# zengxianyu/sketchedit

Measured on NVIDIA H100. Metric: images/sec 256x256 CelebA-HQ generator fwd, higher is better.
Workload: dtype bf16

## Files before the change

### include/sketchedit_b200.h

```cpp
#ifndef SKETCHEDIT_B200_H
#define SKETCHEDIT_B200_H

#ifdef __cplusplus
extern "C" {
#endif

typedef struct se_model se_model;

enum {
  SE_PREC_BF16_TC = 0,
  SE_PREC_FP32_EXACT = 1,
  SE_PREC_FP32_TC = 3
};

enum {
  SE_OPT_USE_CAM = 0,
  SE_OPT_POOL_AVG = 1,
  SE_OPT_NO_MASK_CC = 2,
  SE_OPT_NO_MASK_COARSE = 3,
  SE_OPT_JOINT_TRAIN_INP = 4
};

const char* se_last_error(void);
int se_abi_version(void);
// ... 92 lines not shown
  SE_TAP_DESC_LEN = 10
};
int se_taps_enable(se_model* m, int on);
int se_taps_count(se_model* m);
int se_tap_info(se_model* m, int i, char* name, int name_cap, int* desc, long long* bytes);
int se_tap_copy(se_model* m, int i, void* dst, void* stream);

enum {
  SE_C8_INST = 0,
  SE_C8_TEAMS = 1,
  SE_C8_CLUSTER = 2,
  SE_C8_GRID = 3,
  SE_C8_TOTAL_TILES = 4,
  SE_C8_N = 5, SE_C8_TILES_X = 6, SE_C8_TILES_Y = 7, SE_C8_HO = 8, SE_C8_WO = 9,
  SE_C8_STEP_X = 10, SE_C8_STEP_Y = 11, SE_C8_STEP_IMG = 12,
  SE_C8_CSTEP_X = 13, SE_C8_CSTEP_Y = 14, SE_C8_CSTEP_IMG = 15,
  SE_C8_MODE = 16,
  SE_C8_CPT = 17,
  SE_C8_NCLS = 18,
  SE_C8_A_BUFS = 19, SE_C8_NUM_STAGES = 20,
  SE_C8_OUT_C8 = 21,
  SE_C8_CHOFF = 22, SE_C8_LDO = 23,
  SE_C8_PHANTOM = 24,
  SE_C8_BLK_SPLIT = 25,
  SE_C8_REC_LEN = 26
};
int se_c8_log_enable(int on);
int se_c8_log_count(void);
int se_c8_log_get(int i, char* name, int name_cap, int* rec);
int se_c8_inst_count(void);
enum { SE_C8_INST_NT = 0, SE_C8_INST_F16 = 1, SE_C8_INST_R64 = 2, SE_C8_INST_M64 = 3, SE_C8_INST_R32 = 4, SE_C8_INST_TEAMS = 5,
       SE_C8_INST_LEN = 6 };
int se_c8_inst_info(int i, int* info);

#ifdef __cplusplus
}
#endif
#endif
```

### sketchedit_b200/_lib.py

```python
import ctypes
import os

_HERE = os.path.dirname(os.path.abspath(__file__))
LIB_PATH = os.environ.get("SE_B200_LIB") or os.path.join(_HERE, "libsketchedit_b200.so")

_c_void_p = ctypes.c_void_p
_c_int = ctypes.c_int
_c_char = ctypes.c_char
_c_char_p = ctypes.c_char_p
_fp = ctypes.POINTER(ctypes.c_float)

SIGNATURES = {
    "se_last_error": (_c_char_p, []),
    "se_abi_version": (_c_int, []),
    "se_model_create": (_c_int, [ctypes.POINTER(_c_void_p)]),
    "se_model_destroy": (None, [_c_void_p]),
    "se_model_set_layer": (_c_int, [_c_void_p, _c_char, _c_char_p, _c_void_p, _c_void_p, _c_int, _c_int, _c_int]),
    "se_model_finalize": (_c_int, [_c_void_p]),
    "se_model_set_option": (_c_int, [_c_void_p, _c_int, _c_int]),
    "se_forward_inference": (_c_int, [_c_void_p, _c_void_p, _c_void_p, _c_int, _c_int, _c_int, _c_int,
                                      _c_void_p, _c_void_p, _c_void_p, _c_void_p, _c_void_p, _c_void_p, _c_void_p,
                                      _c_void_p]),
    "se_forward_inference_packed": (_c_int, [_c_void_p, _c_void_p, _c_void_p, _c_int, _c_int, _c_int, _c_int, _c_void_p, _c_void_p]),
    "se_forward_inference_u8": (_c_int, [_c_void_p, _c_void_p, _c_void_p, _c_int, _c_int, _c_int, _c_int, _c_void_p, _c_void_p, _c_void_p]),
# ... 18 lines not shown
    "se_forward_u8_export": (_c_int, [_c_void_p, _c_void_p, _c_void_p, _c_void_p, _c_void_p, _c_int, _c_int, _c_int, _c_int, _c_void_p,
                                      _c_void_p, _c_void_p, _c_void_p, _c_void_p]),
    "se_resize_composite_feather_detail_u8": (_c_int, [_c_void_p, _c_void_p, _c_void_p, _c_void_p, _c_void_p, _c_void_p, _c_void_p,
                                                       _c_void_p, _c_void_p, _c_void_p, _c_void_p, _c_void_p, _c_void_p, _c_int,
                                                       _c_int, _c_void_p, ctypes.POINTER(ctypes.c_longlong), _c_void_p]),
    "se_detail_u8": (_c_int, [_c_void_p, _c_void_p, _c_void_p, _c_int, _c_int, _c_int, _c_void_p, _c_void_p, _c_void_p, _c_void_p,
                              _c_void_p, _c_void_p, _c_void_p, _c_void_p, _c_void_p, _c_void_p, _c_void_p,
                              ctypes.POINTER(ctypes.c_longlong), _c_void_p]),
    "se_feather_u8": (_c_int, [_c_void_p, _c_void_p, _c_void_p, _c_void_p, _c_int, _c_void_p]),
    "se_jpeg_encode_u8": (_c_int, [_c_void_p, _c_void_p, _c_void_p, _c_int, _c_int, _c_int, _c_void_p, _c_void_p, _c_void_p, _c_void_p,
                                   ctypes.POINTER(ctypes.c_longlong), _c_void_p]),
    "se_jpeg_max_bytes": (ctypes.c_longlong, [_c_int, _c_int, _c_int]),
    "se_png_encode_u8": (_c_int, [_c_void_p, _c_void_p, _c_void_p, _c_int, _c_int, _c_int, _c_void_p, _c_void_p, _c_void_p, _c_void_p,
                                  ctypes.POINTER(ctypes.c_longlong), _c_void_p]),
    "se_png_max_bytes": (ctypes.c_longlong, [_c_int, _c_int, _c_int]),
    "se_png_decode_u8": (_c_int, [_c_void_p, _c_void_p, _c_void_p, _c_void_p, _c_void_p, _c_int, _c_void_p, _c_void_p,
                                  _c_void_p, ctypes.POINTER(ctypes.c_longlong), _c_void_p]),
    "se_resize_coeffs": (_c_int, [_c_int, _c_int, _c_void_p, _c_void_p, ctypes.c_longlong]),
    "se_resize_set_table_cache_limit": (_c_int, [ctypes.c_longlong]),
    "se_resize_table_cache_bytes": (ctypes.c_longlong, []),
    "se_last_launch_count": (_c_int, []),
    "se_workspace_bytes": (ctypes.c_longlong, [_c_void_p]),
    "se_timing_enable": (_c_int, [_c_int]),
    "se_timing_report": (_c_int, [_c_char_p, _c_int]),
    "se_taps_enable": (_c_int, [_c_void_p, _c_int]),
    "se_taps_count": (_c_int, [_c_void_p]),
    "se_tap_info": (_c_int, [_c_void_p, _c_int, _c_char_p, _c_int, ctypes.POINTER(_c_int), ctypes.POINTER(ctypes.c_longlong)]),
    "se_tap_copy": (_c_int, [_c_void_p, _c_int, _c_void_p, _c_void_p]),
    "se_c8_log_enable": (_c_int, [_c_int]),
    "se_c8_log_count": (_c_int, []),
    "se_c8_log_get": (_c_int, [_c_int, _c_char_p, _c_int, ctypes.POINTER(_c_int)]),
    "se_c8_inst_count": (_c_int, []),
    "se_c8_inst_info": (_c_int, [_c_int, ctypes.POINTER(_c_int)]),
}

C8_REC = ("inst", "teams", "cluster", "grid", "total_tiles", "N", "tiles_x", "tiles_y", "Ho", "Wo", "step_x", "step_y",
          "step_img", "cstep_x", "cstep_y", "cstep_img", "mode", "cpt", "ncls", "a_bufs", "num_stages", "out_c8", "choff",
          "ldo", "phantom", "blk_split")
C8_INST = ("nt", "f16", "r64", "m64", "r32", "teams")

_lib = None


class SketchEditB200Error(RuntimeError):
    pass


def load():
    global _lib
    if _lib is not None:
        return _lib
    if not os.path.exists(LIB_PATH):
        raise SketchEditB200Error(
            "%s not found. Build it with `python -m sketchedit_b200.build` (nvcc, sm_90a). "
            "There is no CPU or PyTorch fallback for this path." % LIB_PATH)
    lib = ctypes.CDLL(LIB_PATH)
    for name, (res, args) in SIGNATURES.items():
        fn = getattr(lib, name)
        fn.restype = res
        fn.argtypes = args
    _lib = lib
    return lib


def check(rc):
    if rc != 0:
# ... 7 lines not shown
```

### sketchedit_b200/csrc/se_conv_c8.cu

```cuda
#include "se_conv_c8.h"

#include <stdlib.h>

#include <atomic>
#include <map>
#include <mutex>
#include <vector>

#include "../../include/sketchedit_b200.h"
#include "se_tc_device.cuh"

namespace se {

constexpr int C8_TH = 16, C8_TW = 8;
constexpr int C8_CONSUMER_WARPS = 8;
__host__ __device__ constexpr int c8_threads(int teams) { return 32 * C8_CONSUMER_WARPS * teams + 32; }
constexpr int C8_MAX_STAGES = 8;

__device__ __forceinline__ void ring_of(int i, int n, int shift, int& slot, uint32_t& phase) {
  if (shift >= 0) { slot = i & (n - 1); phase = (uint32_t)(i >> shift) & 1u; }
  else { const int qd = i / n; slot = i - qd * n; phase = (uint32_t)qd & 1u; }
}

template <int NT, bool kF16, int R64, int M64, int R32, int TEAMS>
__global__ void __launch_bounds__(c8_threads(TEAMS), 1)
conv_c8_kernel(const __grid_constant__ CUtensorMap tmA, const C8Params p) {
  extern __shared__ __align__(1024) uint8_t smem_raw[];
  uint8_t* smem = reinterpret_cast<uint8_t*>((reinterpret_cast<uintptr_t>(smem_raw) + 1023) & ~uintptr_t(1023));
  constexpr bool kTeams = TEAMS > 1;
  const bool halo = kTeams || p.mode == C8_HALO;
  constexpr int b64_bytes = NT * 128, b32_bytes = NT * 64;
  constexpr int b_bytes = R64 * b64_bytes + R32 * b32_bytes;
  const int stage_a = halo ? 0 : p.a_bytes;
  const int stage_b = p.resident ? 0 : b_bytes;
  const int stage_bytes = stage_a + stage_b;
  const bool staged = !kTeams && stage_bytes > 0;
  uint8_t* sHalo = smem;
  uint8_t* sWres = sHalo + (halo ? p.a_bufs * p.a_bytes : 0);
  uint8_t* sStages = sWres + (p.resident ? p.wres_bytes : 0);
  uint8_t* tail = sStages + (size_t)p.num_stages * stage_bytes;
  uint64_t* full_bar = reinterpret_cast<uint64_t*>(tail);
  uint64_t* empty_bar = full_bar + C8_MAX_STAGES;
  uint64_t* a_full = empty_bar + C8_MAX_STAGES;
  uint64_t* a_empty = a_full + C8_MAX_ABUFS;
  uint64_t* wres_bar = a_empty + C8_MAX_ABUFS;
  float* bias_s = reinterpret_cast<float*>(wres_bar + 2);

  const int warp = threadIdx.x >> 5;
  const int lane = threadIdx.x & 31;
  const bool clustered = !kTeams && p.cluster > 1;
  const uint32_t rank = clustered ? cluster_ctarank() : 0u;
  if (threadIdx.x == 0) {
    for (int i = 0; i < C8_MAX_STAGES; ++i) {
      mbar_init(&full_bar[i], 1);
      mbar_init(&empty_bar[i], C8_CONSUMER_WARPS * p.cluster);
    }
    for (int i = 0; i < C8_MAX_ABUFS; ++i) {
      mbar_init(&a_full[i], 1);
      mbar_init(&a_empty[i], C8_CONSUMER_WARPS);
    }
    mbar_init(wres_bar, 1);
    asm volatile("fence.mbarrier_init.release.cluster;" ::: "memory");
  }
  const int cst_n = NT + 32;
  epi_fill_constants(bias_s, cst_n, p.bias, p.e, threadIdx.x, c8_threads(TEAMS));
  if (clustered) cluster_sync();
  else __syncthreads();

  const int total_tiles = p.N * p.tiles_x * p.tiles_y;
  const int ksteps = kTeams ? 1 : p.ksteps;
  const int first_tile = (int)blockIdx.x - (int)rank;

  if (warp == C8_CONSUMER_WARPS * TEAMS) {
    if (lane == 0) asm volatile("prefetch.tensormap [%0];" ::"l"(reinterpret_cast<uint64_t>(&tmA)) : "memory");
    if (p.resident && elect_one()) {
      mbar_expect_tx(wres_bar, (uint32_t)p.wres_bytes);
      for (int off = 0; off < p.wres_bytes; off += 65536) {
        const int n = min(65536, p.wres_bytes - off);
        bulk_load_1d(sWres + off, p.w + off, (uint32_t)n, wres_bar);
      }
    }
    __syncwarp();
    const int b_split = (b_bytes >> 11) << 10;
    const int b_off = rank ? b_split : 0, b_len = clustered ? (rank ? b_bytes - b_split : b_split) : b_bytes;
    int stage = 0, iter = 0;
    uint32_t phase = 0;
    int tx = blockIdx.x % p.tiles_x, ty = (blockIdx.x / p.tiles_x) % p.tiles_y, img = blockIdx.x / (p.tiles_x * p.tiles_y);
    for (int tile = blockIdx.x; tile - (int)rank < total_tiles; tile += gridDim.x, ++iter) {
      if (tile != (int)blockIdx.x) {
        tx += p.step_x;
        if (tx >= p.tiles_x) { tx -= p.tiles_x; ++ty; }
        ty += p.step_y;
        if (ty >= p.tiles_y) { ty -= p.tiles_y; ++img; }
        img += p.step_img;
      }
      const int x0 = tx * C8_TW, y0 = ty * C8_TH;
      const bool load_a = tile < total_tiles;
      if (halo && load_a) {
        int ab;
        uint32_t aphase;
        ring_of(iter, p.a_bufs, p.a_shift, ab, aphase);
        mbar_wait(&a_empty[ab], aphase ^ 1, 5);
        if (elect_one()) {
// ... 16 lines not shown
            if (!halo && load_a) {
              const int t = ks / p.cpt, ch = ks - t * p.cpt;
              tma_load_4d(st, &tmA, &full_bar[stage], (x0 + p.dx[t]) * 8, y0 + p.dy[t], p.x_cb_off + p.tap_cb[t] + 8 * ch, img);
            }
          }
          __syncwarp();
          if (++stage == p.num_stages) { stage = 0; phase ^= 1; }
        }
      }
    }
  } else {
    const int team = TEAMS > 1 ? warp / C8_CONSUMER_WARPS : 0;
    const int wg = (warp >> 2) & 1, wq = warp & 3;
    const uint32_t smem_base = smem_u32(smem);
    const uint32_t off_wres = halo ? (uint32_t)(p.a_bufs * p.a_bytes) : 0u;
    const uint32_t off_stages = off_wres + (p.resident ? (uint32_t)p.wres_bytes : 0u);
    const uint32_t a_m = (uint32_t)wg * 8u * (uint32_t)p.sbo_bytes;
    const uint32_t n_u64 = p.ntaps * p.n64;
    const int ncls = p.ncls;
    const uint32_t cst_s = smem_u32(bias_s);
    const bool elu = p.e.epi == EPI_GATE_ELU, paired = p.e.paired != 0;
    if (p.resident) mbar_wait(wres_bar, 0, 6);
    auto release = [&](uint64_t* bar) {
      __syncwarp();
      if (lane == 0) mbar_arrive(bar);
    };
    auto release_stage = [&](int s) {
      __syncwarp();
      if (lane == 0) {
        mbar_arrive(&empty_bar[s]);
        if (clustered) mbar_arrive_cluster(&empty_bar[s], rank ^ 1u);
      }
    };
    float acc[NT / 2];
#pragma unroll
    for (int i = 0; i < NT / 2; ++i) acc[i] = 0.0f;
    int stage = 0;
    uint32_t phase = 0;
    const int my_tiles = (first_tile < total_tiles) ? (total_tiles - first_tile + (int)gridDim.x - 1) / (int)gridDim.x : 0;
    const int nv = (my_tiles > team ? (my_tiles - team + TEAMS - 1) / TEAMS : 0) * ncls;
    const bool pingpong = kTeams || (p.resident && ksteps == 1);
    const int bar_wg0 = 2 + 2 * team, bar_wg1 = 1 + 2 * team;
    int riter = team, cls = 0;
    int tx, ty, img;
    {
      const int t0 = (int)blockIdx.x + team * (int)gridDim.x;
      tx = t0 % p.tiles_x; ty = (t0 / p.tiles_x) % p.tiles_y; img = t0 / (p.tiles_x * p.tiles_y);
    }
    for (int v = 0; v < nv; ++v) {
      if (v > 0 && ++cls == ncls) {
        cls = 0;
        riter += TEAMS;
        tx += p.cstep_x;
        if (tx >= p.tiles_x) { tx -= p.tiles_x; ++ty; }
        ty += p.cstep_y;
        if (ty >= p.tiles_y) { ty -= p.tiles_y; ++img; }
        img += p.cstep_img;
      }
      const int tile = (int)blockIdx.x + riter * (int)gridDim.x;
      if (tile >= total_tiles) {
        for (int ks = 0; ks < ksteps; ++ks) {
          mbar_wait(&full_bar[stage], phase, 3);
          release_stage(stage);
          if (++stage == p.num_stages) { stage = 0; phase ^= 1; }
        }
        continue;
      }
      int ab = 0;
      if (halo) {
        uint32_t aph;
        ring_of(riter, p.a_bufs, p.a_shift, ab, aph);
        mbar_wait(&a_full[ab], aph, 7);
      }
      if (pingpong && (wg == 1 || v > 0)) named_bar_sync(wg == 0 ? bar_wg0 : bar_wg1, 256);
      int prev = -1;
      for (int ks = 0; ks < ksteps; ++ks) {
        if (staged) mbar_wait(&full_bar[stage], phase, 3);
        const uint32_t st = smem_base + off_stages + (uint32_t)stage * stage_bytes;
        const uint32_t sB = p.resident ? smem_base + off_wres + (uint32_t)cls * (uint32_t)p.cls_bytes + (uint32_t)ks * b_bytes : st + stage_a;
        const uint32_t sA = (halo ? smem_base + (uint32_t)ab * p.a_bytes : st) + a_m;
        const int ub = cls * C8_CLS_UNITS;
        const int u0 = ub + ks * R64, v0 = ub + (int)n_u64 + ks * R32;
        const uint32_t acc0 = ks ? 1u : 0u;
        wg_fence();
        wg_fence_acc(acc);
#pragma unroll
        for (int j = 0; j < R64; ++j) {
          const uint32_t a0 = sA + p.aoff[u0 + j];
          const uint32_t b0 = sB + (uint32_t)(j * b64_bytes);
#pragma unroll
          for (int k = 0; k < M64; ++k)
            Wgmma<NT, kF16, 0>::mma(acc, wg_desc(a0 + k * p.kstep_bytes, p.lbo_bytes, p.sbo_bytes, WG_SW_NONE),
                                    wg_desc(b0 + 32u * k, 16u, 1024u, WG_SW128), j + k ? 1u : acc0);
        }
#pragma unroll
        for (int j = 0; j < R32; ++j) {
          const uint32_t a0 = sA + p.aoff[v0 + j];
          const uint32_t b0 = sB + (uint32_t)(R64 * b64_bytes + j * b32_bytes);
#pragma unroll
          for (int k = 0; k < 2; ++k)
            Wgmma<NT, kF16, 0>::mma(acc, wg_desc(a0 + k * p.kstep_bytes, p.lbo_bytes, p.sbo_bytes, WG_SW_NONE),
                                    wg_desc(b0 + 32u * k, 16u, 512u, WG_SW64), R64 + j + k ? 1u : acc0);
        }
        wg_commit();
        if (staged) {
          if (prev >= 0) {
            wg_wait<1>();
            release_stage(prev);
          }
          prev = stage;
          if (++stage == p.num_stages) { stage = 0; phase ^= 1; }
        }
      }
      if (pingpong && (wg == 0 || v + 1 < nv)) named_bar_arrive(wg == 0 ? bar_wg1 : bar_wg0, 256);
      wg_wait<0>();
      wg_fence_acc(acc);
      if (prev >= 0) release_stage(prev);
      if (halo && cls == ncls - 1) release(&a_empty[ab]);
      const int ooy = ncls > 1 ? p.cls_ooy[cls] : p.e.ooy, oox = ncls > 1 ? p.cls_oox[cls] : p.e.oox;
      size_t base[2];
      bool ok[2];
#pragma unroll
      for (int h = 0; h < 2; ++h) {
        const int ry = 8 * wg + 2 * wq + h, rx = lane >> 2;
        const int py = ty * C8_TH + ry, px = tx * C8_TW + rx;
        ok[h] = py < p.Ho && px < p.Wo;
        base[h] = epi_pixel_offset(p.e, img, py * p.e.osy + ooy, px * p.e.osx + oox, 2 * (lane & 3));
      }
      if (elu) {
        if (kF16 || paired) conv_epilogue<NT, kF16, true, true>(p.e, cst_s, acc, base, ok, lane);
        else conv_epilogue<NT, false, true, false>(p.e, cst_s, acc, base, ok, lane);
      } else {
        if (kF16 || paired) conv_epilogue<NT, kF16, false, true>(p.e, cst_s, acc, base, ok, lane);
        else conv_epilogue<NT, false, false, false>(p.e, cst_s, acc, base, ok, lane);
      }
    }
  }
  if (clustered) cluster_sync();
}

void fill_epi(const ConvParams& c, int NT, EpiParams* e) {
  e->y = c.y; e->out_c8 = c.out_c8;
  e->Hout = c.Hout; e->Wout = c.Wout; e->ldo = c.ldo; e->choff = c.choff;
  e->osy = c.osy; e->ooy = c.ooy; e->osx = c.osx; e->oox = c.oox;
  e->epi = c.epi; e->scale = c.scale;
  e->Cout = c.Cout; e->NT = NT;
  e->blk_split = c.out_blk_split > 0 ? c.out_blk_split : (1 << 20);
  e->blk_jump = c.out_blk_split > 0 ? c.out_blk_jump : 0;
  e->par_stride = c.out_par_stride > 0 ? c.out_par_stride : (c.ldo >> 2);
  const long long plane = c.out_c8 == 2 ? (long long)(c.Hout / 2) * (c.Wout / 2) : (long long)c.Hout * c.Wout;
  e->blk_stride = (int)(c.out_c8 ? plane * 8 : 8);
  e->goff = gated_goff(c.Cout);
  e->paired = (c.out_c8 != 0 || (((c.ldo | c.choff) & 1) == 0 && c.Cout / 2 == e->goff)) ? 1 : 0;
  e->split_stride = (int)c.out_split_stride;
}
typedef CUresult (*EncodeTiledFn)(CUtensorMap*, CUtensorMapDataType, cuuint32_t, void*, const cuuint64_t*, const cuuint64_t*,
                                  const cuuint32_t*, const cuuint32_t*, CUtensorMapInterleave, CUtensorMapSwizzle,
                                  CUtensorMapL2promotion, CUtensorMapFloatOOBfill);
static EncodeTiledFn c8_encode_fn() {
  static EncodeTiledFn fn = nullptr;
  if (!fn) {
    void* p = nullptr;
    cudaDriverEntryPointQueryResult qres;
    if (cudaGetDriverEntryPoint("cuTensorMapEncodeTiled", &p, cudaEnableDefault, &qres) != cudaSuccess || qres != cudaDriverEntryPointSuccess || !p) return nullptr;
    fn = reinterpret_cast<EncodeTiledFn>(p);
  }
  return fn;
// ... 36 lines not shown
  L->mode = (halo_bytes <= 72 * 1024) ? C8_HALO : C8_PERTAP;
  if (L->mode == C8_HALO) {
    L->HR = HR; L->WR = WR; L->pad_y0 = -mn_y; L->pad_x0 = -mn_x;
  } else {
    L->HR = C8_TH; L->WR = C8_TW; L->pad_y0 = 0; L->pad_x0 = 0;
    L->cb_in = (w.n64 * 64 + w.n32 * 32) / 8;
  }
  L->a_tx_bytes = L->cb_in * L->HR * L->WR * 16;
  L->a_bytes = (L->a_tx_bytes + 1023) / 1024 * 1024;
  L->resident = (wbytes <= kResidentMax) && (2 * L->a_bytes + wbytes <= kSmemBudget);
  if (L->resident && L->mode == C8_HALO) {
    w.r64 = ntaps * w.n64;
    w.r32 = ntaps * w.n32;
  } else if (L->mode == C8_PERTAP || (w.n64 > 0 && w.n32 > 0)) { w.r64 = w.n64; w.r32 = w.n32; }
  else {
    const int unit = w.n64 ? w.NT * 128 : w.NT * 64, total = ntaps * (w.n64 ? w.n64 : w.n32);
    int best = 1;
    for (int k = 1; k <= 8 && k <= total; ++k)
      if (total % k == 0 && k * unit <= 48 * 1024) best = k;
    if (w.n64) { w.r64 = best; w.r32 = 0; } else { w.r64 = 0; w.r32 = best; }
  }
  if (L->mode == C8_PERTAP && w.n32 == 0 && w.n64 > 1 && 2 * (L->a_bytes + w.NT * w.n64 * 128) > kSmemBudget) {
    L->chunks_per_tap = w.n64;
    L->cb_in = 8;
    L->a_tx_bytes = L->cb_in * L->HR * L->WR * 16;
    L->a_bytes = (L->a_tx_bytes + 1023) / 1024 * 1024;
    w.r64 = 1;
  }
  if (L->mode == C8_PERTAP) SE_REQUIRE(tc_ksteps(w) == ntaps * L->chunks_per_tap, "per-tap stages must be whole taps or whole chunks");
  return 0;
}

typedef void (*C8Kernel)(CUtensorMap, C8Params);
struct C8Inst { int nt; bool f16; int r64, m64, r32, teams; C8Kernel fn, fn2; };
#define C8_INST(nt, f16, r64, m64, r32) {nt, f16, r64, m64, r32, 1, conv_c8_kernel<nt, f16, r64, m64, r32, 1>, nullptr}
#define C8_INST2(nt, f16, r64, m64, r32) \
  {nt, f16, r64, m64, r32, 2, conv_c8_kernel<nt, f16, r64, m64, r32, 1>, conv_c8_kernel<nt, f16, r64, m64, r32, 2>}
static const C8Inst kC8Insts[] = {
    C8_INST2(32, false, 0, 0, 9),
    C8_INST2(48, false, 0, 0, 9),
    C8_INST2(48, false, 4, 3, 0),
    C8_INST2(48, false, 5, 3, 0),
    C8_INST2(96, false, 0, 0, 9),
    C8_INST(96, false, 4, 4, 4),
    C8_INST2(96, false, 5, 3, 0),
    C8_INST2(96, false, 9, 3, 0),
    C8_INST(96, false, 3, 3, 0),
    C8_INST(192, false, 1, 3, 0),
    C8_INST(192, false, 1, 4, 0),
    C8_INST(192, false, 1, 4, 1),
    C8_INST2(32, true, 0, 0, 27),
    C8_INST(48, true, 0, 0, 3),
    C8_INST(48, true, 12, 3, 0),
    C8_INST2(48, true, 15, 3, 0),
    C8_INST(96, true, 0, 0, 3),
    C8_INST(96, true, 1, 3, 0),
    C8_INST(96, true, 1, 4, 1),
    C8_INST(96, true, 3, 3, 0),
    C8_INST(192, true, 1, 3, 0),
    C8_INST(192, true, 1, 4, 0),
    C8_INST(192, true, 1, 4, 1),
};
#undef C8_INST
#undef C8_INST2
static const C8Inst* c8_inst(const C8Layer& L, bool f16) {
  const TcWeights& w = L.w;
  const int r64 = w.n64 ? w.r64 : 0, r32 = w.n32 ? w.r32 : 0, m64 = r64 ? L.mmas64 : 0;
  for (const C8Inst& k : kC8Insts)
    if (k.nt == w.NT && k.f16 == f16 && k.r64 == r64 && k.m64 == m64 && k.r32 == r32) return &k;
  return nullptr;
}
static int c8_set_smem_attr(int bytes) {
  for (const C8Inst& k : kC8Insts) {
    SE_CUDA_OK(cudaFuncSetAttribute(k.fn, cudaFuncAttributeMaxDynamicSharedMemorySize, bytes));
    if (k.fn2) SE_CUDA_OK(cudaFuncSetAttribute(k.fn2, cudaFuncAttributeMaxDynamicSharedMemorySize, bytes));
  }
  return 0;
}
int c8_instantiated(const C8Layer& L, bool f16, const std::string& name) {
  const TcWeights& w = L.w;
  SE_REQUIRE(c8_inst(L, f16) != nullptr,
             "layer " + name + (f16 ? " (split-half)" : "") + ": no conv_c8_kernel instantiation for N = " + std::to_string(w.NT) +
                 ", k-step of " + std::to_string(w.n64 ? w.r64 : 0) + " x " + std::to_string(L.mmas64) + " + " +
                 std::to_string(w.n32 ? w.r32 : 0) + " x 2 MMAs (se_conv_c8.cu: kC8Insts)");
  return 0;
}
static void c8_launch_config(cudaLaunchConfig_t* cfg, cudaLaunchAttribute* attr, int grid, int teams, int smem_bytes, int cluster, cudaStream_t stream) {
  *cfg = cudaLaunchConfig_t();
  cfg->gridDim = dim3(grid);
  cfg->blockDim = dim3(c8_threads(teams));
  cfg->dynamicSmemBytes = smem_bytes;
  cfg->stream = stream;
  if (cluster > 1) {
    attr->id = cudaLaunchAttributeClusterDimension;
    attr->val.clusterDim.x = cluster;
    attr->val.clusterDim.y = 1;
    attr->val.clusterDim.z = 1;
    cfg->attrs = attr;
    cfg->numAttrs = 1;
  }
}
static int c8_max_clusters(C8Kernel k, int smem_bytes, int* out) {
  static std::mutex mu;
  static std::map<std::pair<C8Kernel, int>, int> cache;
  std::lock_guard<std::mutex> lock(mu);
  auto it = cache.find({k, smem_bytes});
  if (it == cache.end()) {
    cudaLaunchConfig_t cfg;
    cudaLaunchAttribute attr;
    c8_launch_config(&cfg, &attr, 2 * g_sms, 1, smem_bytes, 2, 0);
    int n = 0;
    SE_CUDA_OK(cudaOccupancyMaxActiveClusters(&n, k, &cfg));
    SE_REQUIRE(n > 0, "no 2-CTA cluster of conv_c8_kernel fits on the device");
    it = cache.emplace(std::make_pair(k, smem_bytes), n).first;
  }
  *out = it->second;
  return 0;
}

struct C8LogEntry { std::string name; int rec[SE_C8_REC_LEN]; };
static std::atomic<bool> g_c8_log{false};
static std::mutex g_c8_log_mu;
static std::vector<C8LogEntry> g_c8_log_recs;
static std::string g_c8_log_label;
bool c8_log_on() { return g_c8_log.load(std::memory_order_relaxed); }
void c8_log_label(const std::string& name) {
  std::lock_guard<std::mutex> lk(g_c8_log_mu);
  g_c8_log_label = name;
}
static void c8_log_append(const C8Params& p, const ConvParams& c, int inst, int teams, int grid, int total_tiles) {
  C8LogEntry e;
  int* r = e.rec;
  r[SE_C8_INST] = inst; r[SE_C8_TEAMS] = teams; r[SE_C8_CLUSTER] = p.cluster; r[SE_C8_GRID] = grid;
  r[SE_C8_TOTAL_TILES] = total_tiles; r[SE_C8_N] = p.N; r[SE_C8_TILES_X] = p.tiles_x; r[SE_C8_TILES_Y] = p.tiles_y;
  r[SE_C8_HO] = p.Ho; r[SE_C8_WO] = p.Wo;
  r[SE_C8_STEP_X] = p.step_x; r[SE_C8_STEP_Y] = p.step_y; r[SE_C8_STEP_IMG] = p.step_img;
  r[SE_C8_CSTEP_X] = p.cstep_x; r[SE_C8_CSTEP_Y] = p.cstep_y; r[SE_C8_CSTEP_IMG] = p.cstep_img;
  r[SE_C8_MODE] = p.mode; r[SE_C8_CPT] = p.cpt; r[SE_C8_NCLS] = p.ncls; r[SE_C8_A_BUFS] = p.a_bufs;
  r[SE_C8_NUM_STAGES] = p.num_stages;
  r[SE_C8_OUT_C8] = c.out_c8; r[SE_C8_CHOFF] = c.choff; r[SE_C8_LDO] = c.ldo;
  r[SE_C8_PHANTOM] = p.cluster > 1 && total_tiles % 2 == 1;
  r[SE_C8_BLK_SPLIT] = c.out_blk_split > 0 ? c.out_blk_split : 0;
  std::lock_guard<std::mutex> lk(g_c8_log_mu);
  e.name = g_c8_log_label;
  g_c8_log_recs.push_back(e);
}

static const int kGroupSmemMax = 222 * 1024;

int c8_configure_group(C8Group* G, int ncls, int ntaps, const int8_t (*dy)[8], const int8_t (*dx)[8], const int* ooy, const int* oox, int Ci, int Cout) {
  if (ncls < 2 || ncls > C8_MAX_CLS || ntaps > 8) return 1;
  int mn_y = 0, mx_y = 0, mn_x = 0, mx_x = 0;
  for (int c = 0; c < ncls; ++c)
    for (int t = 0; t < ntaps; ++t) {
      mn_y = dy[c][t] < mn_y ? dy[c][t] : mn_y; mx_y = dy[c][t] > mx_y ? dy[c][t] : mx_y;
      mn_x = dx[c][t] < mn_x ? dx[c][t] : mn_x; mx_x = dx[c][t] > mx_x ? dx[c][t] : mx_x;
    }
  C8Layer& L = G->geo;
  L = C8Layer();
  TcWeights& w = L.w;
  w.ntaps = ntaps;
  w.n64 = Ci / 64;
  int rem = Ci - 64 * w.n64;
  if (rem > 32) { ++w.n64; rem = 0; }
  w.n32 = rem > 0 ? 1 : 0;
  w.NT = (gated_goff(Cout) + Cout / 2 + 15) / 16 * 16;
  w.n_tiles = 1;
  w.img_bytes = 0;
  w.r64 = ntaps * w.n64;
  w.r32 = ntaps * w.n32;
  L.mmas64 = Ci == 48 ? 3 : 4;
  if (w.r64 + w.r32 > C8_CLS_UNITS) return 1;
  L.mode = C8_HALO;
  L.resident = true;
  L.stem = false;
// ... 95 lines not shown
  SE_REQUIRE(!(L.resident && p.ksteps == 1) || p.a_bufs >= 2, "ping-pong warpgroups need two halo buffers");
  int stages = stage_bytes ? (smem_budget - fixed) / stage_bytes : 1;
  if (stages > C8_MAX_STAGES) stages = C8_MAX_STAGES;
  SE_REQUIRE(stages >= (stage_bytes ? 2 : 1), "shared memory plan does not fit");
  p.num_stages = stages;
  const int smem_bytes = 1024 + fixed + stages * stage_bytes + (2 * C8_MAX_STAGES + 2 * C8_MAX_ABUFS + 2) * 8 + 3 * (p.NT + 32) * 4 + 64;

  EncodeTiledFn enc = c8_encode_fn();
  SE_REQUIRE(enc != nullptr, "cuTensorMapEncodeTiled not available from the driver");
  if (!g_sms) {
    int dev = 0;
    SE_CUDA_OK(cudaGetDevice(&dev));
    SE_CUDA_OK(cudaDeviceGetAttribute(&g_sms, cudaDevAttrMultiProcessorCount, dev));
    SE_CUDA_OK(cudaDeviceGetAttribute(&g_optin, cudaDevAttrMaxSharedMemoryPerBlockOptin, dev));
    { int rc_attr = c8_set_smem_attr(g_optin); if (rc_attr) return rc_attr; }
  }
  SE_REQUIRE(smem_bytes <= g_optin, "shared memory plan exceeds the opt-in limit");

  CUtensorMap tmA;
  {
    cuuint64_t dims[4] = {(cuuint64_t)c.Wi * 8, (cuuint64_t)c.Hi, (cuuint64_t)c.ldx, (cuuint64_t)c.N};
    cuuint64_t strides[3] = {(cuuint64_t)c.Wi * 16, (cuuint64_t)c.Hi * c.Wi * 16, (cuuint64_t)c.ldx * c.Hi * c.Wi * 16};
    cuuint32_t box[4] = {(cuuint32_t)(L.WR * 8), (cuuint32_t)L.HR, (cuuint32_t)L.cb_in, 1};
    cuuint32_t estr[4] = {1, 1, 1, 1};
    CUresult r = enc(&tmA, CU_TENSOR_MAP_DATA_TYPE_BFLOAT16, 4, const_cast<void*>(c.x), dims, strides, box, estr,
                     CU_TENSOR_MAP_INTERLEAVE_NONE, CU_TENSOR_MAP_SWIZZLE_NONE, CU_TENSOR_MAP_L2_PROMOTION_L2_256B,
                     CU_TENSOR_MAP_FLOAT_OOB_FILL_NONE);
    SE_REQUIRE(r == CUDA_SUCCESS, "cuTensorMapEncodeTiled(C8) failed, CUresult=" + std::to_string((int)r));
  }
  const C8Inst* inst = c8_inst(L, p.f16 != 0);
  SE_REQUIRE(inst != nullptr, "no conv_c8_kernel instantiation for the layer's plan (N = " + std::to_string(p.NT) + ")");
  p.cluster = L.resident ? 1 : 2;
  int grid = total_tiles < g_sms ? total_tiles : g_sms;
  const int teams = (inst->teams == 2 && L.resident && p.ksteps == 1 && p.a_bufs >= 4 && total_tiles > grid) ? 2 : 1;
  const C8Kernel kernel = teams == 2 ? inst->fn2 : inst->fn;
  if (p.cluster > 1) {
    int max_clusters = 0;
    { int rc_occ = c8_max_clusters(kernel, smem_bytes, &max_clusters); if (rc_occ) return rc_occ; }
    const int pairs = (total_tiles + 1) / 2;
    grid = 2 * (pairs < max_clusters ? pairs : max_clusters);
  }
  p.step_x = grid % p.tiles_x;
  p.step_y = (grid / p.tiles_x) % p.tiles_y;
  p.step_img = grid / (p.tiles_x * p.tiles_y);
  p.cstep_x = (teams * grid) % p.tiles_x;
  p.cstep_y = (teams * grid / p.tiles_x) % p.tiles_y;
  p.cstep_img = teams * grid / (p.tiles_x * p.tiles_y);
  cudaLaunchConfig_t cfg;
  cudaLaunchAttribute attr;
  c8_launch_config(&cfg, &attr, grid, teams, smem_bytes, p.cluster, stream);
  SE_CUDA_OK(cudaLaunchKernelEx(&cfg, kernel, tmA, p));
  if (c8_log_on()) c8_log_append(p, c, (int)(inst - kC8Insts), teams, grid, total_tiles);
  return 0;
}

}

extern "C" {

int se_c8_log_enable(int on) {
  std::lock_guard<std::mutex> lk(se::g_c8_log_mu);
  se::g_c8_log = on != 0;
  se::g_c8_log_recs.clear();
  se::g_c8_log_label.clear();
  return 0;
}

int se_c8_log_count(void) {
  std::lock_guard<std::mutex> lk(se::g_c8_log_mu);
  return (int)se::g_c8_log_recs.size();
}

int se_c8_log_get(int i, char* name, int name_cap, int* rec) {
  std::lock_guard<std::mutex> lk(se::g_c8_log_mu);
  SE_REQUIRE(i >= 0 && i < (int)se::g_c8_log_recs.size(),
             "launch record index " + std::to_string(i) + " of " + std::to_string(se::g_c8_log_recs.size()));
  const se::C8LogEntry& e = se::g_c8_log_recs[i];
  if (name && name_cap > 0) {
    const size_t n = std::min(e.name.size(), (size_t)name_cap - 1);
    memcpy(name, e.name.data(), n);
    name[n] = 0;
  }
  if (rec) memcpy(rec, e.rec, sizeof(e.rec));
  return 0;
}

int se_c8_inst_count(void) { return (int)(sizeof(se::kC8Insts) / sizeof(se::kC8Insts[0])); }

int se_c8_inst_info(int i, int* info) {
  SE_REQUIRE(i >= 0 && i < se_c8_inst_count() && info, "instantiation index " + std::to_string(i) + " of " + std::to_string(se_c8_inst_count()));
  const se::C8Inst& k = se::kC8Insts[i];
  info[SE_C8_INST_NT] = k.nt; info[SE_C8_INST_F16] = k.f16 ? 1 : 0; info[SE_C8_INST_R64] = k.r64;
  info[SE_C8_INST_M64] = k.m64; info[SE_C8_INST_R32] = k.r32; info[SE_C8_INST_TEAMS] = k.teams;
  return 0;
}

}
```

### sketchedit_b200/csrc/se_conv_c8.h

```cpp
#pragma once
#include "se_common.cuh"
#include "se_conv_tc.h"

namespace se {

enum { C8_HALO = 0, C8_PERTAP = 1 };
constexpr int C8_MAX_ABUFS = 8;
constexpr int C8_MAX_UNITS = 128;

struct C8Layer {
  TcWeights w;
  int mode = C8_HALO;
  bool resident = false;
  bool stem = false;
  int cb_in = 0;
  int mmas64 = 4;
  int HR = 0, WR = 0;
  int pad_y0 = 0, pad_x0 = 0;
  int a_bytes = 0, a_tx_bytes = 0;
  int8_t tap_cb[MAX_TAPS] = {0};
  int chunks_per_tap = 1;
};

constexpr int C8_MAX_CLS = 4;
constexpr int C8_CLS_UNITS = 16;
struct C8Group {
  C8Layer geo;
  int ncls = 0;
  int ntaps = 0;
  int8_t dy[C8_MAX_CLS][8], dx[C8_MAX_CLS][8];
  int ooy[C8_MAX_CLS], oox[C8_MAX_CLS];
  int cls_bytes = 0;
  const void* w_all = nullptr;
};

struct C8Params {
  int N, Ho, Wo;
  int tiles_x, tiles_y;
  int step_x, step_y, step_img;
  int cstep_x, cstep_y, cstep_img;
// ... 29 lines not shown
```

Before: 5087.

## Keep two tiles in flight per consumer warpgroup in c8 ping-pong conv kernel

Adds a PIPE template parameter to the c8 conv kernel so each consumer warpgroup can issue the wgmma chain for the next tile before waiting on and running the epilogue of the current one, using two accumulator register sets. The aim is to hide epilogue latency behind tensor-core work for resident, single-kstep layers whose halo ring is deep enough. Pipelined variants are instantiated for several small-N configurations and picked at launch time. The second accumulator set doubles register pressure and needs one more halo buffer. Logging and ABI hooks report which pipe depth was used.

```diff
diff --git a/include/sketchedit_b200.h b/include/sketchedit_b200.h
--- a/include/sketchedit_b200.h
+++ b/include/sketchedit_b200.h
@@ -148,6 +148,8 @@
 enum { SE_C8_INST_NT = 0, SE_C8_INST_F16 = 1, SE_C8_INST_R64 = 2, SE_C8_INST_M64 = 3, SE_C8_INST_R32 = 4, SE_C8_INST_TEAMS = 5,
        SE_C8_INST_LEN = 6 };
 int se_c8_inst_info(int i, int* info);
+int se_c8_log_pipe(int i, int* pipe);
+int se_c8_inst_pipe(int i, int* pipe);
 
 #ifdef __cplusplus
 }
diff --git a/sketchedit_b200/_lib.py b/sketchedit_b200/_lib.py
--- a/sketchedit_b200/_lib.py
+++ b/sketchedit_b200/_lib.py
@@ -74,6 +74,8 @@
     "se_c8_log_get": (_c_int, [_c_int, _c_char_p, _c_int, ctypes.POINTER(_c_int)]),
     "se_c8_inst_count": (_c_int, []),
     "se_c8_inst_info": (_c_int, [_c_int, ctypes.POINTER(_c_int)]),
+    "se_c8_log_pipe": (_c_int, [_c_int, ctypes.POINTER(_c_int)]),
+    "se_c8_inst_pipe": (_c_int, [_c_int, ctypes.POINTER(_c_int)]),
 }
 
 C8_REC = ("inst", "teams", "cluster", "grid", "total_tiles", "N", "tiles_x", "tiles_y", "Ho", "Wo", "step_x", "step_y",
diff --git a/sketchedit_b200/csrc/se_conv_c8.cu b/sketchedit_b200/csrc/se_conv_c8.cu
--- a/sketchedit_b200/csrc/se_conv_c8.cu
+++ b/sketchedit_b200/csrc/se_conv_c8.cu
@@ -22,19 +22,19 @@
   else { const int qd = i / n; slot = i - qd * n; phase = (uint32_t)qd & 1u; }
 }
 
-template <int NT, bool kF16, int R64, int M64, int R32, int TEAMS>
+template <int NT, bool kF16, int R64, int M64, int R32, int TEAMS, int PIPE>
 __global__ void __launch_bounds__(c8_threads(TEAMS), 1)
 conv_c8_kernel(const __grid_constant__ CUtensorMap tmA, const C8Params p) {
   extern __shared__ __align__(1024) uint8_t smem_raw[];
   uint8_t* smem = reinterpret_cast<uint8_t*>((reinterpret_cast<uintptr_t>(smem_raw) + 1023) & ~uintptr_t(1023));
-  constexpr bool kTeams = TEAMS > 1;
-  const bool halo = kTeams || p.mode == C8_HALO;
+  constexpr bool kPingPongOnly = TEAMS > 1 || PIPE > 1;
+  const bool halo = kPingPongOnly || p.mode == C8_HALO;
   constexpr int b64_bytes = NT * 128, b32_bytes = NT * 64;
   constexpr int b_bytes = R64 * b64_bytes + R32 * b32_bytes;
   const int stage_a = halo ? 0 : p.a_bytes;
   const int stage_b = p.resident ? 0 : b_bytes;
   const int stage_bytes = stage_a + stage_b;
-  const bool staged = !kTeams && stage_bytes > 0;
+  const bool staged = !kPingPongOnly && stage_bytes > 0;
   uint8_t* sHalo = smem;
   uint8_t* sWres = sHalo + (halo ? p.a_bufs * p.a_bytes : 0);
   uint8_t* sStages = sWres + (p.resident ? p.wres_bytes : 0);
@@ -46,9 +46,9 @@
   uint64_t* wres_bar = a_empty + C8_MAX_ABUFS;
   float* bias_s = reinterpret_cast<float*>(wres_bar + 2);
 
-  const int warp = threadIdx.x >> 5;
+  const int warp = PIPE == 2 ? __shfl_sync(0xffffffffu, (int)threadIdx.x >> 5, 0) : (int)threadIdx.x >> 5;
   const int lane = threadIdx.x & 31;
-  const bool clustered = !kTeams && p.cluster > 1;
+  const bool clustered = !kPingPongOnly && p.cluster > 1;
   const uint32_t rank = clustered ? cluster_ctarank() : 0u;
   if (threadIdx.x == 0) {
     for (int i = 0; i < C8_MAX_STAGES; ++i) {
@@ -68,7 +68,7 @@
   else __syncthreads();
 
   const int total_tiles = p.N * p.tiles_x * p.tiles_y;
-  const int ksteps = kTeams ? 1 : p.ksteps;
+  const int ksteps = kPingPongOnly ? 1 : p.ksteps;
   const int first_tile = (int)blockIdx.x - (int)rank;
 
   if (warp == C8_CONSUMER_WARPS * TEAMS) {
@@ -151,91 +151,33 @@
         if (clustered) mbar_arrive_cluster(&empty_bar[s], rank ^ 1u);
       }
     };
-    float acc[NT / 2];
+    auto mma_chain = [&](float (&d)[NT / 2], uint32_t sA, uint32_t sB, int cls, int ks) {
+      const int ub = cls * C8_CLS_UNITS;
+      const int u0 = ub + ks * R64, v0 = ub + (int)n_u64 + ks * R32;
+      const uint32_t acc0 = ks ? 1u : 0u;
+      wg_fence();
+      wg_fence_acc(d);
 #pragma unroll
-    for (int i = 0; i < NT / 2; ++i) acc[i] = 0.0f;
-    int stage = 0;
-    uint32_t phase = 0;
-    const int my_tiles = (first_tile < total_tiles) ? (total_tiles - first_tile + (int)gridDim.x - 1) / (int)gridDim.x : 0;
-    const int nv = (my_tiles > team ? (my_tiles - team + TEAMS - 1) / TEAMS : 0) * ncls;
-    const bool pingpong = kTeams || (p.resident && ksteps == 1);
-    const int bar_wg0 = 2 + 2 * team, bar_wg1 = 1 + 2 * team;
-    int riter = team, cls = 0;
-    int tx, ty, img;
-    {
-      const int t0 = (int)blockIdx.x + team * (int)gridDim.x;
-      tx = t0 % p.tiles_x; ty = (t0 / p.tiles_x) % p.tiles_y; img = t0 / (p.tiles_x * p.tiles_y);
-    }
-    for (int v = 0; v < nv; ++v) {
-      if (v > 0 && ++cls == ncls) {
-        cls = 0;
-        riter += TEAMS;
-        tx += p.cstep_x;
-        if (tx >= p.tiles_x) { tx -= p.tiles_x; ++ty; }
-        ty += p.cstep_y;
-        if (ty >= p.tiles_y) { ty -= p.tiles_y; ++img; }
-        img += p.cstep_img;
-      }
-      const int tile = (int)blockIdx.x + riter * (int)gridDim.x;
-      if (tile >= total_tiles) {
-        for (int ks = 0; ks < ksteps; ++ks) {
-          mbar_wait(&full_bar[stage], phase, 3);
-          release_stage(stage);
-          if (++stage == p.num_stages) { stage = 0; phase ^= 1; }
-        }
-        continue;
-      }
-      int ab = 0;
-      if (halo) {
-        uint32_t aph;
-        ring_of(riter, p.a_bufs, p.a_shift, ab, aph);
-        mbar_wait(&a_full[ab], aph, 7);
-      }
-      if (pingpong && (wg == 1 || v > 0)) named_bar_sync(wg == 0 ? bar_wg0 : bar_wg1, 256);
-      int prev = -1;
-      for (int ks = 0; ks < ksteps; ++ks) {
-        if (staged) mbar_wait(&full_bar[stage], phase, 3);
-        const uint32_t st = smem_base + off_stages + (uint32_t)stage * stage_bytes;
-        const uint32_t sB = p.resident ? smem_base + off_wres + (uint32_t)cls * (uint32_t)p.cls_bytes + (uint32_t)ks * b_bytes : st + stage_a;
-        const uint32_t sA = (halo ? smem_base + (uint32_t)ab * p.a_bytes : st) + a_m;
-        const int ub = cls * C8_CLS_UNITS;
-        const int u0 = ub + ks * R64, v0 = ub + (int)n_u64 + ks * R32;
-        const uint32_t acc0 = ks ? 1u : 0u;
-        wg_fence();
-        wg_fence_acc(acc);
+      for (int j = 0; j < R64; ++j) {
+        const uint32_t a0 = sA + p.aoff[u0 + j];
+        const uint32_t b0 = sB + (uint32_t)(j * b64_bytes);
 #pragma unroll
-        for (int j = 0; j < R64; ++j) {
-          const uint32_t a0 = sA + p.aoff[u0 + j];
-          const uint32_t b0 = sB + (uint32_t)(j * b64_bytes);
+        for (int k = 0; k < M64; ++k)
+          Wgmma<NT, kF16, 0>::mma(d, wg_desc(a0 + k * p.kstep_bytes, p.lbo_bytes, p.sbo_bytes, WG_SW_NONE),
+                                  wg_desc(b0 + 32u * k, 16u, 1024u, WG_SW128), j + k ? 1u : acc0);
+      }
 #pragma unroll
-          for (int k = 0; k < M64; ++k)
-            Wgmma<NT, kF16, 0>::mma(acc, wg_desc(a0 + k * p.kstep_bytes, p.lbo_bytes, p.sbo_bytes, WG_SW_NONE),
-                                    wg_desc(b0 + 32u * k, 16u, 1024u, WG_SW128), j + k ? 1u : acc0);
-        }
+      for (int j = 0; j < R32; ++j) {
+        const uint32_t a0 = sA + p.aoff[v0 + j];
+        const uint32_t b0 = sB + (uint32_t)(R64 * b64_bytes + j * b32_bytes);
 #pragma unroll
-        for (int j = 0; j < R32; ++j) {
-          const uint32_t a0 = sA + p.aoff[v0 + j];
-          const uint32_t b0 = sB + (uint32_t)(R64 * b64_bytes + j * b32_bytes);
-#pragma unroll
-          for (int k = 0; k < 2; ++k)
-            Wgmma<NT, kF16, 0>::mma(acc, wg_desc(a0 + k * p.kstep_bytes, p.lbo_bytes, p.sbo_bytes, WG_SW_NONE),
-                                    wg_desc(b0 + 32u * k, 16u, 512u, WG_SW64), R64 + j + k ? 1u : acc0);
-        }
-        wg_commit();
-        if (staged) {
-          if (prev >= 0) {
-            wg_wait<1>();
-            release_stage(prev);
-          }
-          prev = stage;
-          if (++stage == p.num_stages) { stage = 0; phase ^= 1; }
-        }
-      }
-      if (pingpong && (wg == 0 || v + 1 < nv)) named_bar_arrive(wg == 0 ? bar_wg1 : bar_wg0, 256);
-      wg_wait<0>();
-      wg_fence_acc(acc);
-      if (prev >= 0) release_stage(prev);
-      if (halo && cls == ncls - 1) release(&a_empty[ab]);
+        for (int k = 0; k < 2; ++k)
+          Wgmma<NT, kF16, 0>::mma(d, wg_desc(a0 + k * p.kstep_bytes, p.lbo_bytes, p.sbo_bytes, WG_SW_NONE),
+                                  wg_desc(b0 + 32u * k, 16u, 512u, WG_SW64), R64 + j + k ? 1u : acc0);
+      }
+      wg_commit();
+    };
+    auto epilogue = [&](const float (&d)[NT / 2], int cls, int tx, int ty, int img) {
       const int ooy = ncls > 1 ? p.cls_ooy[cls] : p.e.ooy, oox = ncls > 1 ? p.cls_oox[cls] : p.e.oox;
       size_t base[2];
       bool ok[2];
@@ -247,11 +189,125 @@
         base[h] = epi_pixel_offset(p.e, img, py * p.e.osy + ooy, px * p.e.osx + oox, 2 * (lane & 3));
       }
       if (elu) {
-        if (kF16 || paired) conv_epilogue<NT, kF16, true, true>(p.e, cst_s, acc, base, ok, lane);
-        else conv_epilogue<NT, false, true, false>(p.e, cst_s, acc, base, ok, lane);
+        if (kF16 || paired) conv_epilogue<NT, kF16, true, true>(p.e, cst_s, d, base, ok, lane);
+        else conv_epilogue<NT, false, true, false>(p.e, cst_s, d, base, ok, lane);
       } else {
-        if (kF16 || paired) conv_epilogue<NT, kF16, false, true>(p.e, cst_s, acc, base, ok, lane);
-        else conv_epilogue<NT, false, false, false>(p.e, cst_s, acc, base, ok, lane);
+        if (kF16 || paired) conv_epilogue<NT, kF16, false, true>(p.e, cst_s, d, base, ok, lane);
+        else conv_epilogue<NT, false, false, false>(p.e, cst_s, d, base, ok, lane);
+      }
+    };
+    float acc[PIPE][NT / 2];
+#pragma unroll
+    for (int s = 0; s < PIPE; ++s)
+#pragma unroll
+      for (int i = 0; i < NT / 2; ++i) acc[s][i] = 0.0f;
+    int stage = 0;
+    uint32_t phase = 0;
+    const int my_tiles = (first_tile < total_tiles) ? (total_tiles - first_tile + (int)gridDim.x - 1) / (int)gridDim.x : 0;
+    const int nv = (my_tiles > team ? (my_tiles - team + TEAMS - 1) / TEAMS : 0) * ncls;
+    const bool pingpong = kPingPongOnly || (p.resident && ksteps == 1);
+    const int bar_wg0 = 2 + 2 * team, bar_wg1 = 1 + 2 * team;
+    struct VTile { int riter, cls, tx, ty, img; };
+    VTile t;
+    {
+      const int t0 = (int)blockIdx.x + team * (int)gridDim.x;
+      t = {team, 0, t0 % p.tiles_x, (t0 / p.tiles_x) % p.tiles_y, t0 / (p.tiles_x * p.tiles_y)};
+    }
+    auto advance = [&](VTile& u) {
+      if (++u.cls < ncls) return;
+      u.cls = 0;
+      u.riter += TEAMS;
+      u.tx += p.cstep_x;
+      if (u.tx >= p.tiles_x) { u.tx -= p.tiles_x; ++u.ty; }
+      u.ty += p.cstep_y;
+      if (u.ty >= p.tiles_y) { u.ty -= p.tiles_y; ++u.img; }
+      u.img += p.cstep_img;
+    };
+    if constexpr (PIPE == 1) {
+      for (int v = 0; v < nv; ++v) {
+        if (v > 0) advance(t);
+        const int tile = (int)blockIdx.x + t.riter * (int)gridDim.x;
+        if (tile >= total_tiles) {
+          for (int ks = 0; ks < ksteps; ++ks) {
+            mbar_wait(&full_bar[stage], phase, 3);
+            release_stage(stage);
+            if (++stage == p.num_stages) { stage = 0; phase ^= 1; }
+          }
+          continue;
+        }
+        int ab = 0;
+        if (halo) {
+          uint32_t aph;
+          ring_of(t.riter, p.a_bufs, p.a_shift, ab, aph);
+          mbar_wait(&a_full[ab], aph, 7);
+        }
+        if (pingpong && (wg == 1 || v > 0)) named_bar_sync(wg == 0 ? bar_wg0 : bar_wg1, 256);
+        int prev = -1;
+        for (int ks = 0; ks < ksteps; ++ks) {
+          if (staged) mbar_wait(&full_bar[stage], phase, 3);
+          const uint32_t st = smem_base + off_stages + (uint32_t)stage * stage_bytes;
+          const uint32_t sB = p.resident ? smem_base + off_wres + (uint32_t)t.cls * (uint32_t)p.cls_bytes + (uint32_t)ks * b_bytes : st + stage_a;
+          const uint32_t sA = (halo ? smem_base + (uint32_t)ab * p.a_bytes : st) + a_m;
+          mma_chain(acc[0], sA, sB, t.cls, ks);
+          if (staged) {
+            if (prev >= 0) {
+              wg_wait<1>();
+              release_stage(prev);
+            }
+            prev = stage;
+            if (++stage == p.num_stages) { stage = 0; phase ^= 1; }
+          }
+        }
+        if (pingpong && (wg == 0 || v + 1 < nv)) named_bar_arrive(wg == 0 ? bar_wg1 : bar_wg0, 256);
+        wg_wait<0>();
+        wg_fence_acc(acc[0]);
+        if (prev >= 0) release_stage(prev);
+        if (halo && t.cls == ncls - 1) release(&a_empty[ab]);
+        epilogue(acc[0], t.cls, t.tx, t.ty, t.img);
+      }
+    } else {
+      auto issue = [&](float (&d)[NT / 2], const VTile& u, int v) {
+        int ab;
+        uint32_t aph;
+        ring_of(u.riter, p.a_bufs, p.a_shift, ab, aph);
+        mbar_wait(&a_full[ab], aph, 7);
+        if (wg == 1 || v > 0) named_bar_sync(wg == 0 ? bar_wg0 : bar_wg1, 256);
+        mma_chain(d, smem_base + (uint32_t)ab * p.a_bytes + a_m, smem_base + off_wres + (uint32_t)u.cls * (uint32_t)p.cls_bytes, u.cls, 0);
+        if (wg == 0 || v + 1 < nv) named_bar_arrive(wg == 0 ? bar_wg1 : bar_wg0, 256);
+      };
+      auto finish = [&](float (&cur)[NT / 2]) {
+        wg_fence_acc(cur);
+        if (t.cls == ncls - 1) {
+          int ab;
+          uint32_t aph;
+          ring_of(t.riter, p.a_bufs, p.a_shift, ab, aph);
+          release(&a_empty[ab]);
+        }
+        epilogue(cur, t.cls, t.tx, t.ty, t.img);
+      };
+      auto step = [&](float (&cur)[NT / 2], float (&nxt)[NT / 2], int v) {
+        VTile n = t;
+        advance(n);
+        issue(nxt, n, v + 1);
+        wg_wait<1>();
+        finish(cur);
+        t = n;
+      };
+      if (nv > 0) {
+        issue(acc[0], t, 0);
+        int v = 0;
+        for (; v + 2 < nv; v += 2) {
+          step(acc[0], acc[1], v);
+          step(acc[1], acc[0], v + 1);
+        }
+        if (v + 1 < nv) {
+          step(acc[0], acc[1], v);
+          wg_wait<0>();
+          finish(acc[1]);
+        } else {
+          wg_wait<0>();
+          finish(acc[0]);
+        }
       }
     }
   }
@@ -354,15 +410,19 @@
 }
 
 typedef void (*C8Kernel)(CUtensorMap, C8Params);
-struct C8Inst { int nt; bool f16; int r64, m64, r32, teams; C8Kernel fn, fn2; };
-#define C8_INST(nt, f16, r64, m64, r32) {nt, f16, r64, m64, r32, 1, conv_c8_kernel<nt, f16, r64, m64, r32, 1>, nullptr}
+struct C8Inst { int nt; bool f16; int r64, m64, r32, teams, pipe; C8Kernel fn[2][2]; };
+#define C8_K(nt, f16, r64, m64, r32, teams, pipe) conv_c8_kernel<nt, f16, r64, m64, r32, teams, pipe>
+#define C8_INST(nt, f16, r64, m64, r32) {nt, f16, r64, m64, r32, 1, 1, {{C8_K(nt, f16, r64, m64, r32, 1, 1), nullptr}, {nullptr, nullptr}}}
 #define C8_INST2(nt, f16, r64, m64, r32) \
-  {nt, f16, r64, m64, r32, 2, conv_c8_kernel<nt, f16, r64, m64, r32, 1>, conv_c8_kernel<nt, f16, r64, m64, r32, 2>}
+  {nt, f16, r64, m64, r32, 2, 1, {{C8_K(nt, f16, r64, m64, r32, 1, 1), nullptr}, {C8_K(nt, f16, r64, m64, r32, 2, 1), nullptr}}}
+#define C8_INST2P(nt, f16, r64, m64, r32)                                                     \
+  {nt, f16, r64, m64, r32, 2, 2, {{C8_K(nt, f16, r64, m64, r32, 1, 1), C8_K(nt, f16, r64, m64, r32, 1, 2)}, \
+                                  {C8_K(nt, f16, r64, m64, r32, 2, 1), C8_K(nt, f16, r64, m64, r32, 2, 2)}}}
 static const C8Inst kC8Insts[] = {
-    C8_INST2(32, false, 0, 0, 9),
-    C8_INST2(48, false, 0, 0, 9),
-    C8_INST2(48, false, 4, 3, 0),
-    C8_INST2(48, false, 5, 3, 0),
+    C8_INST2P(32, false, 0, 0, 9),
+    C8_INST2P(48, false, 0, 0, 9),
+    C8_INST2P(48, false, 4, 3, 0),
+    C8_INST2P(48, false, 5, 3, 0),
     C8_INST2(96, false, 0, 0, 9),
     C8_INST(96, false, 4, 4, 4),
     C8_INST2(96, false, 5, 3, 0),
@@ -371,10 +431,10 @@
     C8_INST(192, false, 1, 3, 0),
     C8_INST(192, false, 1, 4, 0),
     C8_INST(192, false, 1, 4, 1),
-    C8_INST2(32, true, 0, 0, 27),
+    C8_INST2P(32, true, 0, 0, 27),
     C8_INST(48, true, 0, 0, 3),
     C8_INST(48, true, 12, 3, 0),
-    C8_INST2(48, true, 15, 3, 0),
+    C8_INST2P(48, true, 15, 3, 0),
     C8_INST(96, true, 0, 0, 3),
     C8_INST(96, true, 1, 3, 0),
     C8_INST(96, true, 1, 4, 1),
@@ -383,8 +443,10 @@
     C8_INST(192, true, 1, 4, 0),
     C8_INST(192, true, 1, 4, 1),
 };
+#undef C8_K
 #undef C8_INST
 #undef C8_INST2
+#undef C8_INST2P
 static const C8Inst* c8_inst(const C8Layer& L, bool f16) {
   const TcWeights& w = L.w;
   const int r64 = w.n64 ? w.r64 : 0, r32 = w.n32 ? w.r32 : 0, m64 = r64 ? L.mmas64 : 0;
@@ -393,10 +455,9 @@
   return nullptr;
 }
 static int c8_set_smem_attr(int bytes) {
-  for (const C8Inst& k : kC8Insts) {
-    SE_CUDA_OK(cudaFuncSetAttribute(k.fn, cudaFuncAttributeMaxDynamicSharedMemorySize, bytes));
-    if (k.fn2) SE_CUDA_OK(cudaFuncSetAttribute(k.fn2, cudaFuncAttributeMaxDynamicSharedMemorySize, bytes));
-  }
+  for (const C8Inst& k : kC8Insts)
+    for (C8Kernel fn : {k.fn[0][0], k.fn[0][1], k.fn[1][0], k.fn[1][1]})
+      if (fn) SE_CUDA_OK(cudaFuncSetAttribute(fn, cudaFuncAttributeMaxDynamicSharedMemorySize, bytes));
   return 0;
 }
 int c8_instantiated(const C8Layer& L, bool f16, const std::string& name) {
@@ -440,7 +501,7 @@
   return 0;
 }
 
-struct C8LogEntry { std::string name; int rec[SE_C8_REC_LEN]; };
+struct C8LogEntry { std::string name; int rec[SE_C8_REC_LEN]; int pipe; };
 static std::atomic<bool> g_c8_log{false};
 static std::mutex g_c8_log_mu;
 static std::vector<C8LogEntry> g_c8_log_recs;
@@ -450,7 +511,7 @@
   std::lock_guard<std::mutex> lk(g_c8_log_mu);
   g_c8_log_label = name;
 }
-static void c8_log_append(const C8Params& p, const ConvParams& c, int inst, int teams, int grid, int total_tiles) {
+static void c8_log_append(const C8Params& p, const ConvParams& c, int inst, int teams, int pipe, int grid, int total_tiles) {
   C8LogEntry e;
   int* r = e.rec;
   r[SE_C8_INST] = inst; r[SE_C8_TEAMS] = teams; r[SE_C8_CLUSTER] = p.cluster; r[SE_C8_GRID] = grid;
@@ -463,6 +524,7 @@
   r[SE_C8_OUT_C8] = c.out_c8; r[SE_C8_CHOFF] = c.choff; r[SE_C8_LDO] = c.ldo;
   r[SE_C8_PHANTOM] = p.cluster > 1 && total_tiles % 2 == 1;
   r[SE_C8_BLK_SPLIT] = c.out_blk_split > 0 ? c.out_blk_split : 0;
+  e.pipe = pipe;
   std::lock_guard<std::mutex> lk(g_c8_log_mu);
   e.name = g_c8_log_label;
   g_c8_log_recs.push_back(e);
@@ -624,8 +686,13 @@
   SE_REQUIRE(inst != nullptr, "no conv_c8_kernel instantiation for the layer's plan (N = " + std::to_string(p.NT) + ")");
   p.cluster = L.resident ? 1 : 2;
   int grid = total_tiles < g_sms ? total_tiles : g_sms;
-  const int teams = (inst->teams == 2 && L.resident && p.ksteps == 1 && p.a_bufs >= 4 && total_tiles > grid) ? 2 : 1;
-  const C8Kernel kernel = teams == 2 ? inst->fn2 : inst->fn;
+  const bool pingpong = L.resident && p.ksteps == 1;
+  const int teams = (inst->teams == 2 && pingpong && p.a_bufs >= 4 && total_tiles > grid) ? 2 : 1;
+  const int pipe = (inst->pipe == 2 && pingpong && p.a_bufs >= c8_ring_min(teams, 2) + 1) ? 2 : 1;
+  SE_REQUIRE(p.a_bufs >= c8_ring_min(teams, pipe), "halo ring too shallow for the launch form");
+  const C8Kernel kernel = inst->fn[teams - 1][pipe - 1];
+  SE_REQUIRE(kernel != nullptr, "conv_c8_kernel has no form with " + std::to_string(teams) + " team(s) and " + std::to_string(pipe) +
+                                    " tile(s) in flight per warpgroup for this layer");
   if (p.cluster > 1) {
     int max_clusters = 0;
     { int rc_occ = c8_max_clusters(kernel, smem_bytes, &max_clusters); if (rc_occ) return rc_occ; }
@@ -642,7 +709,7 @@
   cudaLaunchAttribute attr;
   c8_launch_config(&cfg, &attr, grid, teams, smem_bytes, p.cluster, stream);
   SE_CUDA_OK(cudaLaunchKernelEx(&cfg, kernel, tmA, p));
-  if (c8_log_on()) c8_log_append(p, c, (int)(inst - kC8Insts), teams, grid, total_tiles);
+  if (c8_log_on()) c8_log_append(p, c, (int)(inst - kC8Insts), teams, pipe, grid, total_tiles);
   return 0;
 }
 
@@ -687,4 +754,18 @@
   return 0;
 }
 
-}
+int se_c8_log_pipe(int i, int* pipe) {
+  std::lock_guard<std::mutex> lk(se::g_c8_log_mu);
+  SE_REQUIRE(i >= 0 && i < (int)se::g_c8_log_recs.size() && pipe,
+             "launch record index " + std::to_string(i) + " of " + std::to_string(se::g_c8_log_recs.size()));
+  *pipe = se::g_c8_log_recs[i].pipe;
+  return 0;
+}
+
+int se_c8_inst_pipe(int i, int* pipe) {
+  SE_REQUIRE(i >= 0 && i < se_c8_inst_count() && pipe, "instantiation index " + std::to_string(i) + " of " + std::to_string(se_c8_inst_count()));
+  *pipe = se::kC8Insts[i].pipe;
+  return 0;
+}
+
+}
diff --git a/sketchedit_b200/csrc/se_conv_c8.h b/sketchedit_b200/csrc/se_conv_c8.h
--- a/sketchedit_b200/csrc/se_conv_c8.h
+++ b/sketchedit_b200/csrc/se_conv_c8.h
@@ -6,6 +6,7 @@
 
 enum { C8_HALO = 0, C8_PERTAP = 1 };
 constexpr int C8_MAX_ABUFS = 8;
+constexpr int c8_ring_min(int teams, int pipe) { return teams + pipe - 1; }
 constexpr int C8_MAX_UNITS = 128;
 
 struct C8Layer {
```

After: 5234 (median of 6 runs). 2.9% higher.
